# JuliaSmoothOptimizers/LinearOperators.jl

Hardware: AMD Instinct MI355X
Metric: mul! GB/s (frac HBM peak) at n=10^8 fp64; L-BFGS apply/s, 1/2/4/8 GPU (higher is better)
Workload: dtype f64; 1 GPU; opHouseholder(h) 5-arg mul!(res,H,v,1,0), n=100000000 fp64 per GPU (configs[1]); n_per_gpu=100000000, algorithmic_bytes_per_elt=40, devices_visible=1

## Files before the change

linearoperators.jl_amd/csrc/api_ctx.hip:

```cpp
#include "common.h"
#include <vector>

namespace mxlo {
static thread_local char g_err[512] = "";
void set_error(const char *fmt, ...) {
  va_list ap;
  va_start(ap, fmt);
  vsnprintf(g_err, sizeof(g_err), fmt, ap);
  va_end(ap);
}
}

using namespace mxlo;

MXLO_API const char *mxlo_version(void) { return "mxlo 0.1.0 (gfx950)"; }

MXLO_API const char *mxlo_status_string(int32_t s) {
  switch (s) {
    case MXLO_OK: return "ok";
    case MXLO_EINVAL: return "invalid argument";
    case MXLO_ESHAPE: return "shape mismatch";
    case MXLO_EHIP: return "HIP runtime error";
    case MXLO_ENOMEM: return "out of device memory";
    case MXLO_ESTATE: return "wrong variant for this operator state";
// ... 359 lines not shown
MXLO_API int32_t mxlo_ctx_info(mxlo_ctx *ctx, int64_t info[4]) {
  MXLO_REQUIRE(ctx && info, MXLO_EINVAL, "ctx/info is NULL");
  info[0] = ctx->device;
  info[1] = ctx->num_cu;
  info[2] = (int64_t)sizeof(double) * (kMaxRedCols * kMaxRedBlocks + kScalarSlots);
  info[3] = kMaxRedCols;
  return MXLO_OK;
}

MXLO_API int32_t mxlo_ctx_tune(mxlo_ctx *ctx, const char *key, int64_t value) {
  MXLO_REQUIRE(ctx && key, MXLO_EINVAL, "ctx/key is NULL");
  if (!strcmp(key, "blocks_per_cu")) {
    MXLO_REQUIRE(value >= 0 && value <= 64, MXLO_EINVAL, "blocks_per_cu out of range");
    ctx->tune.blocks_per_cu = (int)value;
  } else if (!strcmp(key, "nt_min_bytes")) {
    MXLO_REQUIRE(value >= 0, MXLO_EINVAL, "nt_min_bytes out of range");
    ctx->tune.nt_min_bytes = value;
  } else if (!strcmp(key, "red_blocks_per_cu")) {
    MXLO_REQUIRE(value >= 1 && value * ctx->num_cu <= kMaxRedBlocks, MXLO_EINVAL,
                 "red_blocks_per_cu out of range");
    ctx->tune.red_blocks_per_cu = (int)value;
  } else if (!strcmp(key, "graph_direct_max")) {
    MXLO_REQUIRE(value >= 0 && value <= 4096, MXLO_EINVAL, "graph_direct_max must be in 0..4096 (0: always hipGraphLaunch)");
    ctx->tune.graph_direct_max = (int)value;
  } else if (!strcmp(key, "house_fused")) {
    ctx->tune.house_fused = value != 0;
  } else if (!strcmp(key, "cherm_two_pass")) {
    ctx->tune.cherm_two_pass = value != 0;
  } else if (!strcmp(key, "house_inline_n")) {
    MXLO_REQUIRE(value >= 0, MXLO_EINVAL, "house_inline_n out of range");
    ctx->tune.house_inline_n = value;
  } else if (!strcmp(key, "house_reverse")) {
    ctx->tune.house_reverse = value != 0;
  } else if (!strcmp(key, "lbfgs_inv_mode")) {
    MXLO_REQUIRE(value == MXLO_INV_TWOPASS || value == MXLO_INV_REFORDER, MXLO_EINVAL,
                 "lbfgs_inv_mode must be MXLO_INV_TWOPASS or MXLO_INV_REFORDER");
    ctx->tune.lbfgs_inv_mode = (int)value;
  } else if (!strcmp(key, "gemm_tile")) {
    MXLO_REQUIRE(value == 0 || value == 32 || value == 64 || value == 128 || value == -1, MXLO_EINVAL,
                 "gemm_tile must be 0 (auto), 32, 64, 128 or -1 (generic kernel)");
    ctx->tune.gemm_tile = (int)value;
  } else if (!strcmp(key, "extend_tiles_per_block")) {
    MXLO_REQUIRE(value >= 0 && value <= 1024, MXLO_EINVAL, "extend_tiles_per_block must be in 0..1024 (0 = auto)");
    ctx->tune.extend_tiles_per_block = (int)value;
  } else if (!strcmp(key, "fuse_finalize")) {
    MXLO_REQUIRE(value == 0 || value == 1, MXLO_EINVAL, "fuse_finalize must be 0 or 1");
    ctx->tune.fuse_finalize = (int)value;
  } else if (!strcmp(key, "combine_blocks_per_cu")) {
    MXLO_REQUIRE(value >= 0 && value <= 64, MXLO_EINVAL, "combine_blocks_per_cu out of range");
    ctx->tune.combine_blocks_per_cu = (int)value;
  } else if (!strcmp(key, "qn_fused_max_grid")) {
    MXLO_REQUIRE(value >= 1 && value <= kQnfMaxGrid, MXLO_EINVAL, "qn_fused_max_grid must be in 1..256");
    ctx->tune.qn_fused_max_grid = (int)value;
  } else if (!strcmp(key, "qn_fused_batch12")) {
    MXLO_REQUIRE(value == 0 || value == 1, MXLO_EINVAL, "qn_fused_batch12 must be 0 or 1");
    ctx->tune.qn_fused_batch12 = (int)value;
  } else if (!strcmp(key, "qn_fused_small")) {
    MXLO_REQUIRE(value == 0 || value == 1, MXLO_EINVAL, "qn_fused_small must be 0 or 1");
    ctx->tune.qn_fused_small = (int)value;
  } else if (!strcmp(key, "qn_persist")) {
    MXLO_REQUIRE(value == 0 || value == 1, MXLO_EINVAL, "qn_persist must be 0 or 1");
    ctx->tune.qn_persist = (int)value;
  } else if (!strcmp(key, "qn_persist_min_n")) {
    MXLO_REQUIRE(value >= 1, MXLO_EINVAL, "qn_persist_min_n must be >= 1");
    ctx->tune.qn_persist_min_n = value;
  } else if (!strcmp(key, "qn_persist_max_bytes")) {
// ... 206 lines not shown
```

linearoperators.jl_amd/csrc/common.h:

```cpp
#pragma once
#include <hip/hip_runtime.h>
#include <atomic>

#include <cstdarg>
#include <cstdint>
#include <cstdio>
#include <cstdlib>
#include <cstring>
#include <initializer_list>
#include <type_traits>
#include <utility>
#include <vector>

#include "../../include/mxlo.h"

#define MXLO_API extern "C" __attribute__((visibility("default")))

namespace mxlo {

constexpr int kBlock = 256;
constexpr int kWave = 64;
constexpr int kMaxRedCols = 128;
constexpr int kQnfMaxCols = 40, kQnfMaxGrid = 256;
constexpr int kQnfSlots = kQnfMaxCols * kQnfMaxGrid;
// ... 62 lines not shown
  } while (0)

inline bool mxlo_trace_on() {
  static const bool on = getenv("MXLO_TRACE") != nullptr;
  return on;
}
#define MXLO_LAUNCH_CHECK()                                                                      \
  do {                                                                                           \
    ++mxlo::api_counters().n_launch;                                                             \
    if (mxlo_trace_on()) {                                                                       \
      fprintf(stderr, "[mxlo] launched %s:%d ... ", __FILE__, __LINE__);                         \
      fflush(stderr);                                                                            \
      (void)hipDeviceSynchronize();                                                              \
      fprintf(stderr, "done\n");                                                                 \
    }                                                                                            \
    hipError_t e__ = hipGetLastError();                                                          \
    if (e__ != hipSuccess) {                                                                     \
      mxlo::set_error("kernel launch failed: %s (%s:%d)", hipGetErrorString(e__), __FILE__,      \
                      __LINE__);                                                                 \
      return MXLO_EHIP;                                                                          \
    }                                                                                            \
  } while (0)

struct Tune {
  int blocks_per_cu = 0;
  int extend_tiles_per_block = 0;
  int64_t nt_min_bytes = 256ll << 20;
  int red_blocks_per_cu = 4;
  int graph_direct_max = 16;
  int house_fused_per_cu = 2;
  int house_fused = 1;
  int cherm_two_pass = 0;
  int house_reverse = 1;
  int64_t house_inline_n = 1ll << 23;
  int lbfgs_inv_mode = MXLO_INV_TWOPASS;
  int dots_max_nc = 20;
  int gemm_tile = 0;
  int fuse_finalize = 1;
  int combine_blocks_per_cu = 0;
  int qn_fused_max_grid = 256;
  int qn_fused_batch12 = 1;
  int qn_fused_small = 1;
  int qn_persist = 1;
  int64_t qn_persist_min_n = 1ll << 19;
  int64_t qn_persist_max_bytes = 448ll << 20;
  int qn_persist_reverse = 1;
  int qn_persist_prefetch = 0;
  int qn_persist_lds = 1;
  int qn_persist_lds_pad = 0;
  int64_t qn_persist_min_bytes = 32ll << 20;
  int herm_order = 1;
  int herm_nt = -1;
  int64_t herm_dp_min_bytes = 96ll << 20;
  int64_t herm_nt_min_bytes = 384ll << 20;
  int herm_poll_sleep = 4;
  int herm_strip = 0;
  int herm_lds_pad = 0;
  int herm_single = 1;
  int64_t herm_single_max_n = 0;
  int64_t herm_single_max_bytes = 112ll << 20;
  int kron_fuse = 1;
  int gemv_n_rows = 1;
  int gemvb_n_rows = 1;
  int gemvb_t_lds = 1;
  int combine_reverse = 0;
  int push_wide = 1;
// ... 213 lines not shown
template <typename T>
inline int64_t common_head(std::initializer_list<const void *> ptrs) {
  int64_t mis = -1;
  for (const void *p : ptrs) {
    if (!p) continue;
    int64_t m = (int64_t)((uintptr_t)p & 15u);
    if (m % (int64_t)sizeof(T)) return -1;
    if (mis < 0) mis = m;
    else if (mis != m) return -1;
  }
  if (mis <= 0) return 0;
  return (16 - mis) / (int64_t)sizeof(T);
}

inline int grid_for(const mxlo_ctx *ctx, int64_t work_items, int64_t items_per_block, int per_cu) {
  int64_t need = (work_items + items_per_block - 1) / items_per_block;
  int64_t g = need;
  if (per_cu > 0) {
    const int64_t cap = (int64_t)ctx->num_cu * per_cu;
    if (g > cap) g = cap;
  }
  if (g > 0x7fffffffLL) g = 0x7fffffffLL;
  return (int)(g < 1 ? 1 : g);
}

bool qn_generation(const mxlo_qn *h, int64_t *gen);

int32_t finalize_and_reduce(mxlo_ctx *ctx, int ncols, int nblocks, double *out_dev);
int32_t finalize_and_post(mxlo_ctx *ctx, int ncols, int nblocks, double *out_dev, double *post_dev, unsigned long long seq,
                          const double *extra_src, int extra_n);
int32_t allreduce_hook(mxlo_ctx *ctx, double *dev, int64_t count);
template <typename T>
int32_t panel_dots(mxlo_ctx *ctx, const T *const *cols_host, int ncols, const T *x, int64_t n,
                   double *out_dev);
template <typename T>
int32_t panel_dots_partials(mxlo_ctx *ctx, const T *const *cols_host, int ncols, const T *x, int64_t n, int *nblocks);
template <typename T>
int32_t panel_dots2(mxlo_ctx *ctx, const T *const *cols, int ncols, const T *x1, const T *x2, int64_t n_padded,
                    double *out1, double *out2);
struct PushExtras {
  const double *cp_src = nullptr;
  double *cp_dst = nullptr;
  int cp_n = 0;
  double *post = nullptr;
  unsigned long long post_seq = 0;
};
template <typename T>
int32_t panel_push_pass(mxlo_ctx *ctx, const T *const *cols, int ncols, int slot, int slot_src, const T *x1,
                        const T *x2, int64_t n, int64_t n_padded, T *st1, T *st2, T *stb, double sq, double *out1,
                        double *out2, double *out_x1x2, double *out_x2x2, double *out_bb, double *out_x1x1 = nullptr,
                        const PushExtras *extras = nullptr);

}
```

linearoperators.jl_amd/csrc/leaves.hip:

```cpp
#include "common.h"
#include "stream_kernels.h"

using namespace mxlo;

#define CHECK_COMMON(name)                                                                       \
  MXLO_REQUIRE(ctx != nullptr, MXLO_EINVAL, name ": ctx is NULL");                               \
  MXLO_REQUIRE(dtype == MXLO_F64 || dtype == MXLO_F32, MXLO_EINVAL, name ": bad dtype %d", dtype)

static inline double eff_beta(int32_t dtype, int32_t flags, double beta) {
  return beta_is_f64(dtype == MXLO_F64 ? 8 : 4, flags) ? beta : (double)(float)beta;
}
static inline double eff_alpha(int32_t dtype, int32_t flags, double alpha) {
  return alpha_is_f64(dtype == MXLO_F64 ? 8 : 4, flags) ? alpha : (double)(float)alpha;
}

template <typename T>
static int32_t fill(mxlo_ctx *ctx, T *p, int64_t n, T c) {
  if (n <= 0) return MXLO_OK;
  if (c == T(0)) {
    MXLO_HIP(hipMemsetAsync(p, 0, sizeof(T) * (size_t)n, ctx->stream));
    return MXLO_OK;
  }
  return launch_map<T, 0, false, false>(ctx, p, (const T *)nullptr, (const T *)nullptr, n,
                                        FillOp<T>{c});
// ... 152 lines not shown
template <typename T>
static int32_t ones_mul_t(mxlo_ctx *ctx, T *res, int64_t nrow, const T *v, int64_t ncol,
                          double alpha, double beta, int32_t flags) {
  double *sum = ctx->scalars;
  if (ncol > 0) {
    const int grid = grid_for(ctx, ncol, kBlock * 8, ctx->tune.red_blocks_per_cu);
    hipLaunchKernelGGL((sum_kernel<T>), dim3(grid), dim3(kBlock), 0, ctx->stream, v, ncol,
                       ctx->partials);
    MXLO_LAUNCH_CHECK();
    MXLO_TRY(finalize_and_reduce(ctx, 1, grid, sum));
  } else {
    MXLO_HIP(hipMemsetAsync(sum, 0, sizeof(double), ctx->stream));
  }
  MXLO_TRY(allreduce_hook(ctx, sum, 1));
  return dispatch_ab<T>(beta, flags, [&]<typename CA, typename CB, bool B0>() -> int32_t {
    OnesOp<T, CA, CB, B0> op{(CA)alpha, (CB)beta, sum, (CA)0};
    return launch_map<T, 0, !B0, false>(ctx, res, (const T *)nullptr, (const T *)nullptr, nrow, op);
  });
}

MXLO_API int32_t mxlo_ones_mul(mxlo_ctx *ctx, int32_t dtype, void *res, int64_t nrow,
                               const void *v, int64_t ncol, double alpha, double beta,
                               int32_t flags) {
  CHECK_COMMON("mxlo_ones_mul");
  MXLO_DEVICE_GUARD(ctx);
  MXLO_REQUIRE(nrow >= 0 && ncol >= 0, MXLO_ESHAPE, "mxlo_ones_mul: negative size");
  alpha = eff_alpha(dtype, flags, alpha);
  beta = eff_beta(dtype, flags, beta);
  if (dtype == MXLO_F64)
    return ones_mul_t<double>(ctx, (double *)res, nrow, (const double *)v, ncol, alpha, beta, flags);
  return ones_mul_t<float>(ctx, (float *)res, nrow, (const float *)v, ncol, alpha, beta, flags);
}

template <typename T>
static int32_t householder_apply_t(mxlo_ctx *ctx, T *res, const T *h, const T *v, int64_t n,
                                   double alpha, double beta, int32_t flags, const double *dot) {
  const bool rev = ctx->tune.house_reverse != 0;
  return dispatch_ab<T>(beta, flags, [&]<typename CA, typename CB, bool B0>() -> int32_t {
    HouseholderOp<T, CA, CB, B0> op{(CA)alpha, (CB)beta, dot, T(0)};
    if (rev) return launch_map<T, 2, !B0, true>(ctx, res, h, v, n, op);
    return launch_map<T, 2, !B0, false>(ctx, res, h, v, n, op);
  });
}

namespace {
template <typename T, typename CA, typename CB, bool BETA0, int VPT, bool ALIGNED>
__global__ void __launch_bounds__(kBlock)
householder_fused_kernel(T *__restrict__ res, const T *__restrict__ h, const T *__restrict__ v, int64_t n, CA alpha,
                         CB beta, unsigned long long *__restrict__ slots, unsigned long long ticks,
                         unsigned *__restrict__ fault, int drop) {
  constexpr int VEC = Vec16<T>::N;
  using V = typename Vec16<T>::type;
  const int tid = threadIdx.x, G = (int)gridDim.x, b = (int)blockIdx.x;
  unsigned long long *epoch = slots + 2 * kFusedSlots;
  const unsigned e = (unsigned)__hip_atomic_load(epoch, __ATOMIC_RELAXED, __HIP_MEMORY_SCOPE_AGENT) & 1u;
  unsigned long long *mine = slots + e * kFusedSlots, *other = slots + (1u - e) * kFusedSlots;
  for (int i = b + tid * G; i < kFusedSlots; i += G * kBlock)
    __hip_atomic_store(other + i, kSlotEmpty, __ATOMIC_RELAXED, __HIP_MEMORY_SCOPE_AGENT);

  T hh[VPT][VEC], vv[VPT][VEC];
  double acc = 0.0;
  const int64_t base = (int64_t)b * kBlock * VPT * VEC;
#pragma unroll
  for (int q = 0; q < VPT; ++q) {
    const int64_t i = base + ((int64_t)q * kBlock + tid) * VEC;
    if (ALIGNED && i + VEC <= n) {
      const V a = *reinterpret_cast<const V *>(h + i), c = *reinterpret_cast<const V *>(v + i);
#pragma unroll
      for (int k = 0; k < VEC; ++k) { hh[q][k] = a[k]; vv[q][k] = c[k]; }
    } else {
#pragma unroll
      for (int k = 0; k < VEC; ++k) {
        hh[q][k] = i + k < n ? h[i + k] : T(0);
        vv[q][k] = i + k < n ? v[i + k] : T(0);
      }
// ... 73 lines not shown
      else if (vpt == 4) go.template operator()<4, true>();
      else if (vpt == 8) go.template operator()<8, true>();
      else go.template operator()<16, true>();
    } else {
      if (vpt == 2) go.template operator()<2, false>();
      else if (vpt == 4) go.template operator()<4, false>();
      else if (vpt == 8) go.template operator()<8, false>();
      else go.template operator()<16, false>();
    }
    *launched = fits;
    if (!fits) return MXLO_OK;
    MXLO_LAUNCH_CHECK();
    return MXLO_OK;
  });
}

template <typename T>
static int32_t householder_t(mxlo_ctx *ctx, T *res, const T *h, const T *v, int64_t n,
                             double alpha, double beta, int32_t flags) {
  if (ctx->tune.house_fused && !ctx->allreduce && n > 0 && ctx->fault_dev) {
    MXLO_TRY(fused_fault_check(ctx));
  }
  if (ctx->tune.house_fused && !ctx->allreduce && n > 0 && ctx->fault_dev) {
    const int64_t cap = std::min<int64_t>((int64_t)ctx->num_cu * (ctx->tune.house_fused_per_cu >= 2 ? 2 : 1), kFusedSlots);
    const int64_t cap1 = std::min<int64_t>(ctx->num_cu, kFusedSlots);
    const int vpt = fused_grid<T>(n, 2) <= 16 ? 2 : (fused_grid<T>(n, 4) <= 32 ? 4 : (fused_grid<T>(n, 8) <= cap1 ? 8 : 16));
    if (fused_grid<T>(n, vpt) <= cap) {
      bool launched = false;
      const int32_t st = householder_fused_t<T>(ctx, res, h, v, n, alpha, beta, flags, vpt, &launched);
      if (st != MXLO_OK || launched) return st;
    }
  }
  const T *cols[1] = {h};
  if (!ctx->allreduce && n >= 1 && n <= ctx->tune.house_inline_n) {
    int nb = 0;
    MXLO_TRY(panel_dots_partials<T>(ctx, cols, 1, v, n, &nb));
    const bool rev = ctx->tune.house_reverse != 0;
    return dispatch_ab<T>(beta, flags, [&]<typename CA, typename CB, bool B0>() -> int32_t {
      HouseholderPartialsOp<T, CA, CB, B0> op{(CA)alpha, (CB)beta, ctx->partials, nb, T(0)};
      if (rev) return launch_map<T, 2, !B0, true>(ctx, res, h, v, n, op);
      return launch_map<T, 2, !B0, false>(ctx, res, h, v, n, op);
    });
  }
  double *dot = ctx->scalars;
  MXLO_TRY(panel_dots<T>(ctx, cols, 1, v, n, dot));
  return householder_apply_t<T>(ctx, res, h, v, n, alpha, beta, flags, dot);
}

MXLO_API int32_t mxlo_dot(mxlo_ctx *ctx, int32_t dtype, const void *a, const void *b, int64_t n,
                          double *out_dev) {
  CHECK_COMMON("mxlo_dot");
  MXLO_DEVICE_GUARD(ctx);
  MXLO_REQUIRE(n >= 0 && out_dev && (n == 0 || (a && b)), MXLO_EINVAL, "mxlo_dot: bad argument");
  if (dtype == MXLO_F64) {
    const double *cols[1] = {(const double *)a};
    return panel_dots<double>(ctx, cols, 1, (const double *)b, n, out_dev);
  }
  const float *cols[1] = {(const float *)a};
  return panel_dots<float>(ctx, cols, 1, (const float *)b, n, out_dev);
}

MXLO_API int32_t mxlo_householder_apply(mxlo_ctx *ctx, int32_t dtype, void *res, const void *h,
                                        const void *v, int64_t n, double alpha, double beta,
                                        int32_t flags, const double *dot_dev) {
  CHECK_COMMON("mxlo_householder_apply");
  MXLO_DEVICE_GUARD(ctx);
  MXLO_REQUIRE(n >= 0 && dot_dev && (n == 0 || (res && h && v)), MXLO_EINVAL,
               "mxlo_householder_apply: bad argument");
  MXLO_TRY(stage_alias(ctx, res, n * (dtype == MXLO_F64 ? 8 : 4), &v, n * (dtype == MXLO_F64 ? 8 : 4), true,
                       "mxlo_householder_apply"));
  alpha = eff_alpha(dtype, flags, alpha);
  beta = eff_beta(dtype, flags, beta);
  if (dtype == MXLO_F64)
    return householder_apply_t<double>(ctx, (double *)res, (const double *)h, (const double *)v, n,
                                       alpha, beta, flags, dot_dev);
  return householder_apply_t<float>(ctx, (float *)res, (const float *)h, (const float *)v, n, alpha,
                                    beta, flags, dot_dev);
}

// ... 681 lines not shown
```

linearoperators.jl_amd/csrc/reductions.hip:

```cpp
#include "common.h"

namespace mxlo {

constexpr int kFuseMaxCols = 4;
constexpr int kFuseMaxGrid = 64;

template <typename T, int NC>
struct ColPtrs {
  const T *p[NC];
};

__device__ __forceinline__ double wave_sum(double v) {
#if defined(__HIP_DEVICE_COMPILE__)
  {
    const int lo = __double2loint(v), hi = __double2hiint(v);
    const auto slo = __builtin_amdgcn_permlane32_swap(lo, lo, false, false);
    const auto shi = __builtin_amdgcn_permlane32_swap(hi, hi, false, false);
    v += __hiloint2double((int)shi[1], (int)slo[1]);
  }
  {
    const int lo = __double2loint(v), hi = __double2hiint(v);
    const auto slo = __builtin_amdgcn_permlane16_swap(lo, lo, false, false);
    const auto shi = __builtin_amdgcn_permlane16_swap(hi, hi, false, false);
    v += __hiloint2double((int)shi[1], (int)slo[1]);
// ... 103 lines not shown
#pragma unroll
  for (int c = 0; c < NC; ++c) {
    const double s = wave_sum(acc[c]);
    if (lane == 0) lds[wave][c] = s;
  }
  __syncthreads();
  if (tid < NC) {
    const double s = ((lds[0][tid] + lds[1][tid]) + (lds[2][tid] + lds[3][tid]));
    if constexpr (FUSE) store_agent(partials + (int64_t)tid * kMaxRedBlocks + blockIdx.x, s);
    else partials[(int64_t)tid * kMaxRedBlocks + blockIdx.x] = s;
  }
  if constexpr (FUSE) {
    __shared__ int last;
    __threadfence();
    __syncthreads();
    if (tid == 0) last = atomicAdd(ticket, 1u) == gridDim.x - 1;
    __syncthreads();
    if (!last) return;
    __threadfence();
    const int nblocks = (int)gridDim.x;
#pragma unroll 1
    for (int c = 0; c < NC; ++c) {
      const double *p = partials + (int64_t)c * kMaxRedBlocks;
      double s = 0.0;
      for (int i = tid; i < nblocks; i += kBlock) s += load_agent(p + i);
      s = wave_sum(s);
      __syncthreads();
      if (lane == 0) lds[wave][0] = s;
      __syncthreads();
      if (tid == 0) out[c] = (lds[0][0] + lds[1][0]) + (lds[2][0] + lds[3][0]);
    }
    if (tid == 0) __hip_atomic_store(ticket, 0u, __ATOMIC_RELAXED, __HIP_MEMORY_SCOPE_AGENT);
  }
}

__global__ void __launch_bounds__(kBlock)
finalize_kernel(const double *__restrict__ partials, int nblocks, double *__restrict__ out) {
  const int c = blockIdx.x, tid = threadIdx.x;
  const double *p = partials + (int64_t)c * kMaxRedBlocks;
  double s = 0.0;
  for (int i = tid; i < nblocks; i += kBlock) s += p[i];
  s = wave_sum(s);
  __shared__ double lds[kBlock / kWave];
  if ((tid & 63) == 0) lds[tid >> 6] = s;
  __syncthreads();
  if (tid == 0) out[c] = (lds[0] + lds[1]) + (lds[2] + lds[3]);
}

int32_t finalize_and_reduce(mxlo_ctx *ctx, int ncols, int nblocks, double *out_dev) {
  hipLaunchKernelGGL(finalize_kernel, dim3(ncols), dim3(kBlock), 0, ctx->stream, ctx->partials,
                     nblocks, out_dev);
  MXLO_LAUNCH_CHECK();
  return MXLO_OK;
}

__global__ void __launch_bounds__(kBlock)
finalize_post_kernel(const double *__restrict__ partials, int nblocks, double *__restrict__ out, double *post,
                     unsigned long long seq, const double *__restrict__ extra_src, int extra_n) {
  const int c = blockIdx.x, tid = threadIdx.x;
  auto post_pair = [&](int i, double v) {
    unsigned long long *slot = reinterpret_cast<unsigned long long *>(post) + 2 * i;
    __hip_atomic_store(slot, (unsigned long long)__double_as_longlong(v), __ATOMIC_RELAXED, __HIP_MEMORY_SCOPE_SYSTEM);
    __threadfence_system();
    __hip_atomic_store(slot + 1, seq, __ATOMIC_RELEASE, __HIP_MEMORY_SCOPE_SYSTEM);
  };
  const double *p = partials + (int64_t)c * kMaxRedBlocks;
// ... 31 lines not shown
template <typename T, int VEC, int NC, bool XVEC>
static int32_t launch_dots(mxlo_ctx *ctx, const T *const *cols, const T *x, int64_t head,
                           int64_t nvec, int64_t n, int *nblocks_out, double *fused_out = nullptr) {
  ColPtrs<T, NC> cp;
  for (int c = 0; c < NC; ++c) cp.p[c] = cols[c];
  constexpr int UNROLL = NC <= 2 ? 4 : (NC <= 6 ? 2 : 1);
  const bool nt = (int64_t)sizeof(T) * n * (NC + 1) >= ctx->tune.nt_min_bytes;
  const int per_cu = (nt && NC <= 2 && ctx->tune.red_blocks_per_cu > 1) ? 1 : ctx->tune.red_blocks_per_cu;
  const int grid = grid_for(ctx, nvec, (int64_t)kBlock * UNROLL, per_cu);
  if constexpr (NC <= kFuseMaxCols) {
    if (fused_out && grid <= kFuseMaxGrid) {
      if (nt)
        hipLaunchKernelGGL((panel_dots_kernel<T, VEC, NC, UNROLL, XVEC, true, true>), dim3(grid), dim3(kBlock), 0,
                           ctx->stream, cp, x, head, nvec, n, ctx->partials, ctx->ticket, fused_out);
      else
        hipLaunchKernelGGL((panel_dots_kernel<T, VEC, NC, UNROLL, XVEC, false, true>), dim3(grid), dim3(kBlock), 0,
                           ctx->stream, cp, x, head, nvec, n, ctx->partials, ctx->ticket, fused_out);
      MXLO_LAUNCH_CHECK();
      *nblocks_out = 0;
      return MXLO_OK;
    }
  }
  if (nt)
    hipLaunchKernelGGL((panel_dots_kernel<T, VEC, NC, UNROLL, XVEC, true>), dim3(grid), dim3(kBlock), 0,
                       ctx->stream, cp, x, head, nvec, n, ctx->partials);
  else
    hipLaunchKernelGGL((panel_dots_kernel<T, VEC, NC, UNROLL, XVEC, false>), dim3(grid), dim3(kBlock), 0,
                       ctx->stream, cp, x, head, nvec, n, ctx->partials);
  MXLO_LAUNCH_CHECK();
  *nblocks_out = grid;
  return MXLO_OK;
}

#define DOTS_CASE(NCV)                                                                           \
  case NCV:                                                                                      \
    if (vec && xvec) return launch_dots<T, Vec16<T>::N, NCV, true>(ctx, cols, x, head, nvec, n, nb, fo); \
    if (vec) return launch_dots<T, Vec16<T>::N, NCV, false>(ctx, cols, x, head, nvec, n, nb, fo); \
    break;

template <typename T>
static int32_t dots_chunk(mxlo_ctx *ctx, const T *const *cols, int nc, const T *x, int64_t n,
                          int *nb, double *fo = nullptr) {
  constexpr int VEC = Vec16<T>::N;
  int64_t head = 0;
  bool vec = n >= 4 * VEC;
  if (vec) {
    int64_t mis = -1;
    for (int c = 0; c < nc && vec; ++c) {
      int64_t m = (int64_t)((uintptr_t)cols[c] & 15u);
      if (m % (int64_t)sizeof(T)) vec = false;
      else if (mis < 0) mis = m;
      else if (mis != m) vec = false;
    }
    if (vec) head = mis == 0 ? 0 : (16 - mis) / (int64_t)sizeof(T);
  }
  const int64_t nvec = vec ? (n - head) / VEC : n;
  const bool xvec = vec && ((((uintptr_t)(x + head)) & 15u) == 0);
  switch (nc) {
    DOTS_CASE(1) DOTS_CASE(2) DOTS_CASE(3) DOTS_CASE(4) DOTS_CASE(5) DOTS_CASE(6) DOTS_CASE(7)
    DOTS_CASE(8) DOTS_CASE(9) DOTS_CASE(10) DOTS_CASE(11) DOTS_CASE(12) DOTS_CASE(13)
    DOTS_CASE(14) DOTS_CASE(15) DOTS_CASE(16) DOTS_CASE(17) DOTS_CASE(18) DOTS_CASE(19)
    DOTS_CASE(20)
    default: break;
  }
  switch (nc) {
    case 1: return launch_dots<T, 1, 1, false>(ctx, cols, x, 0, n, n, nb, fo);
    case 2: return launch_dots<T, 1, 2, false>(ctx, cols, x, 0, n, n, nb, fo);
    case 3: return launch_dots<T, 1, 3, false>(ctx, cols, x, 0, n, n, nb, fo);
    case 4: return launch_dots<T, 1, 4, false>(ctx, cols, x, 0, n, n, nb, fo);
    default: break;
  }
  set_error("dots_chunk: unsupported column count %d", nc);
  return MXLO_EINVAL;
}

template <typename T>
int32_t panel_dots(mxlo_ctx *ctx, const T *const *cols, int ncols, const T *x, int64_t n,
                   double *out_dev) {
  MXLO_REQUIRE(ncols >= 0 && ncols <= kMaxRedCols, MXLO_EINVAL, "panel_dots: %d columns", ncols);
  if (ncols == 0) return MXLO_OK;
  if (n <= 0) {
    MXLO_HIP(hipMemsetAsync(out_dev, 0, sizeof(double) * ncols, ctx->stream));
    return allreduce_hook(ctx, out_dev, ncols);
  }
  constexpr int VEC = Vec16<T>::N;
  int done = 0;
  while (done < ncols) {
    int nc = ncols - done;
    if (nc > ctx->tune.dots_max_nc) nc = ctx->tune.dots_max_nc;
    bool vec = n >= 4 * VEC;
    int64_t mis = -1;
    for (int c = 0; c < nc && vec; ++c) {
      int64_t m = (int64_t)((uintptr_t)cols[done + c] & 15u);
      if (m % (int64_t)sizeof(T) || (mis >= 0 && mis != m)) vec = false;
      mis = m;
    }
    if (!vec && nc > 4) nc = 4;
    int nb = 0;
    const bool fuse = ctx->tune.fuse_finalize && done == 0 && nc == ncols && nc <= kFuseMaxCols;
    MXLO_TRY(dots_chunk<T>(ctx, cols + done, nc, x, n, &nb, fuse ? out_dev : nullptr));
    if (nb > 0) MXLO_TRY(finalize_and_reduce(ctx, nc, nb, out_dev + done));
    done += nc;
  }
  return allreduce_hook(ctx, out_dev, ncols);
}

template <typename T>
int32_t panel_dots_partials(mxlo_ctx *ctx, const T *const *cols, int ncols, const T *x, int64_t n, int *nblocks) {
  MXLO_REQUIRE(ncols >= 1 && ncols <= 4 && n >= 1, MXLO_EINVAL, "panel_dots_partials: bad arguments");
  return dots_chunk<T>(ctx, cols, ncols, x, n, nblocks, nullptr);
}
template int32_t panel_dots_partials<double>(mxlo_ctx *, const double *const *, int, const double *, int64_t, int *);
template int32_t panel_dots_partials<float>(mxlo_ctx *, const float *const *, int, const float *, int64_t, int *);

template <typename T, int NC, int UNROLL, bool NT>
__global__ void __launch_bounds__(kBlock)
panel_dots2_kernel(ColPtrs<T, NC> cols, const T *__restrict__ x1, const T *__restrict__ x2, int64_t nvec,
                   double *__restrict__ partials) {
  constexpr int VEC = Vec16<T>::N;
  using V = typename Vec16<T>::type;
  const int tid = threadIdx.x;
  double a1[NC], a2[NC];
#pragma unroll
  for (int c = 0; c < NC; ++c) a1[c] = a2[c] = 0.0;
  auto ld = [&](const T *p, int64_t i) -> V {
    return NT ? __builtin_nontemporal_load(reinterpret_cast<const V *>(p) + i) : reinterpret_cast<const V *>(p)[i];
  };
  constexpr int64_t CHUNK = (int64_t)kBlock * UNROLL;
  const int64_t nchunks = (nvec + CHUNK - 1) / CHUNK;
  for (int64_t ch = blockIdx.x; ch < nchunks; ch += gridDim.x) {
    const int64_t base = ch * CHUNK + tid;
    V xv1[UNROLL], xv2[UNROLL], cv[UNROLL][NC];
    bool ok[UNROLL];
#pragma unroll
    for (int u = 0; u < UNROLL; ++u) {
      const int64_t i = base + (int64_t)u * kBlock;
      ok[u] = i < nvec;
      if (ok[u]) {
        xv1[u] = ld(x1, i);
        xv2[u] = ld(x2, i);
#pragma unroll
        for (int c = 0; c < NC; ++c) cv[u][c] = ld(cols.p[c], i);
      }
    }
#pragma unroll
    for (int u = 0; u < UNROLL; ++u) {
// ... 280 lines not shown
    }
    hipLaunchKernelGGL(finalize_map_kernel, dim3(2 * NC + 4), dim3(kBlock), 0, ctx->stream, ctx->partials, grid, M);
  };
  switch (ncols) {
    case 1: go.template operator()<1>(); break;
    case 2: go.template operator()<2>(); break;
    case 3: go.template operator()<3>(); break;
    case 4: go.template operator()<4>(); break;
    case 5: go.template operator()<5>(); break;
    case 6: go.template operator()<6>(); break;
    case 7: go.template operator()<7>(); break;
    case 8: go.template operator()<8>(); break;
    case 9: go.template operator()<9>(); break;
    case 10: go.template operator()<10>(); break;
    default: go.template operator()<kPushMaxNC>(); break;
  }
  MXLO_LAUNCH_CHECK();
  return MXLO_OK;
}

template int32_t panel_push_pass<double>(mxlo_ctx *, const double *const *, int, int, int, const double *, const double *,
                                         int64_t, int64_t, double *, double *, double *, double, double *, double *,
                                         double *, double *, double *, double *, const PushExtras *);
template int32_t panel_push_pass<float>(mxlo_ctx *, const float *const *, int, int, int, const float *, const float *,
                                        int64_t, int64_t, float *, float *, float *, double, double *, double *, double *,
                                        double *, double *, double *, const PushExtras *);

template int32_t panel_dots2<double>(mxlo_ctx *, const double *const *, int, const double *, const double *, int64_t,
                                     double *, double *);
template int32_t panel_dots2<float>(mxlo_ctx *, const float *const *, int, const float *, const float *, int64_t,
                                    double *, double *);

template int32_t panel_dots<double>(mxlo_ctx *, const double *const *, int, const double *, int64_t,
                                    double *);
template int32_t panel_dots<float>(mxlo_ctx *, const float *const *, int, const float *, int64_t,
                                   double *);

}
```

linearoperators.jl_amd/csrc/stream_kernels.h:

```cpp
#pragma once
#include "common.h"

namespace mxlo {

template <bool NT, typename V>
__device__ __forceinline__ V ldg(const V *p) {
  if constexpr (NT) return __builtin_nontemporal_load(p);
  else return *p;
}
template <bool NT, typename V>
__device__ __forceinline__ void stg(V *p, V v) {
  if constexpr (NT) __builtin_nontemporal_store(v, p);
  else *p = v;
}

template <typename T, int VEC>
struct VecOf {
  using type = T;
};
template <>
struct VecOf<double, 2> {
  using type = f64x2;
};
template <>
// ... 109 lines not shown
  constexpr int VEC = Vec16<T>::N;
  const int64_t head0 = common_head<T>({res, NIN >= 1 ? in0 : nullptr, NIN >= 2 ? in1 : nullptr});
  const int64_t streamed = (int64_t)sizeof(T) * n * (1 + NIN + (READ_RES ? 1 : 0));
  const bool nt = streamed >= ctx->tune.nt_min_bytes;
  auto grid_of = [&](int64_t items) {
    const int64_t need = (items + (int64_t)kBlock * kStreamUnroll - 1) / ((int64_t)kBlock * kStreamUnroll);
    int64_t g = need;
    if (ctx->tune.blocks_per_cu > 0) {
      const int64_t cap = (int64_t)ctx->num_cu * ctx->tune.blocks_per_cu;
      if (g > cap) g = cap;
    }
    if (g > 0x7fffffffLL) g = 0x7fffffffLL;
    return (int)(g < 1 ? 1 : g);
  };
  if (head0 >= 0 && n >= 4 * VEC) {
    const int64_t head = head0 < n ? head0 : n;
    const int64_t nvec = (n - head) / VEC;
    const int grid = grid_of(nvec);
    if (nt)
      hipLaunchKernelGGL((map_kernel<T, VEC, kStreamUnroll, NIN, READ_RES, REVERSE, true, Op>), dim3(grid),
                         dim3(kBlock), 0, ctx->stream, res, in0, in1, head, nvec, n, op);
    else
      hipLaunchKernelGGL((map_kernel<T, VEC, kStreamUnroll, NIN, READ_RES, REVERSE, false, Op>), dim3(grid),
                         dim3(kBlock), 0, ctx->stream, res, in0, in1, head, nvec, n, op);
  } else {
    const int grid = grid_of(n);
    hipLaunchKernelGGL((map_kernel<T, 1, kStreamUnroll, NIN, READ_RES, REVERSE, false, Op>), dim3(grid),
                       dim3(kBlock), 0, ctx->stream, res, in0, in1, (int64_t)0, n, n, op);
  }
  MXLO_LAUNCH_CHECK();
  return MXLO_OK;
}

template <typename CA, typename CB>
using Wider = std::conditional_t<(sizeof(CA) >= sizeof(CB)), CA, CB>;

template <typename T, typename CA, typename CB, bool BETA0>
__device__ __forceinline__ T fin_ab(CA t, CB b, T r) {
  if constexpr (BETA0) return (T)t;
  else {
    using P = Wider<CA, CB>;
    return (T)((P)t + (P)(b * (CB)r));
  }
}

template <typename T, typename CA, typename CB, bool BETA0>
struct DiagOp {
  CA a;
  CB b;
  __device__ void init() {}
  __device__ T operator()(T d, T v, T r) const { return fin_ab<T, CA, CB, BETA0>((a * (CA)d) * (CA)v, b, r); }
};
template <typename T, typename CA, typename CB, bool BETA0>
struct DiagScalarOp {
  CA a;
  CB b;
  const T *dptr;
  CA ad;
  __device__ void init() { ad = a * (CA)(*dptr); }
  __device__ T operator()(T v, T, T r) const { return fin_ab<T, CA, CB, BETA0>(ad * (CA)v, b, r); }
};
template <typename T, typename CA, typename CB, bool BETA0>
struct AxpbyOp {
  CA a;
  CB b;
  __device__ void init() {}
// ... 80 lines not shown
```

Before: 6428 GB/s.

## Keep Householder dot-pass tail cache-resident for the reversed update pass

```diff
diff --git a/linearoperators.jl_amd/csrc/api_ctx.hip b/linearoperators.jl_amd/csrc/api_ctx.hip
--- a/linearoperators.jl_amd/csrc/api_ctx.hip
+++ b/linearoperators.jl_amd/csrc/api_ctx.hip
@@ -415,6 +415,13 @@
     ctx->tune.house_inline_n = value;
   } else if (!strcmp(key, "house_reverse")) {
     ctx->tune.house_reverse = value != 0;
+  } else if (!strcmp(key, "house_tail_bytes")) {
+    MXLO_REQUIRE(value >= 0, MXLO_EINVAL, "house_tail_bytes out of range");
+    ctx->tune.house_tail_bytes = value;
+  } else if (!strcmp(key, "house_tail_store_nt")) {
+    ctx->tune.house_tail_store_nt = value != 0;
+  } else if (!strcmp(key, "house_tail_dots_nt")) {
+    ctx->tune.house_tail_dots_nt = value != 0;
   } else if (!strcmp(key, "lbfgs_inv_mode")) {
     MXLO_REQUIRE(value == MXLO_INV_TWOPASS || value == MXLO_INV_REFORDER, MXLO_EINVAL,
                  "lbfgs_inv_mode must be MXLO_INV_TWOPASS or MXLO_INV_REFORDER");
diff --git a/linearoperators.jl_amd/csrc/common.h b/linearoperators.jl_amd/csrc/common.h
--- a/linearoperators.jl_amd/csrc/common.h
+++ b/linearoperators.jl_amd/csrc/common.h
@@ -118,6 +118,9 @@
   int house_fused = 1;
   int cherm_two_pass = 0;
   int house_reverse = 1;
+  int64_t house_tail_bytes = 128ll << 20;
+  int house_tail_store_nt = 1;
+  int house_tail_dots_nt = 0;
   int64_t house_inline_n = 1ll << 23;
   int lbfgs_inv_mode = MXLO_INV_TWOPASS;
   int dots_max_nc = 20;
@@ -397,9 +400,10 @@
 int32_t allreduce_hook(mxlo_ctx *ctx, double *dev, int64_t count);
 template <typename T>
 int32_t panel_dots(mxlo_ctx *ctx, const T *const *cols_host, int ncols, const T *x, int64_t n,
-                   double *out_dev);
-template <typename T>
-int32_t panel_dots_partials(mxlo_ctx *ctx, const T *const *cols_host, int ncols, const T *x, int64_t n, int *nblocks);
+                   double *out_dev, int64_t nc1_tail_bytes = 0);
+template <typename T>
+int32_t panel_dots_partials(mxlo_ctx *ctx, const T *const *cols_host, int ncols, const T *x, int64_t n, int *nblocks,
+                            int64_t nc1_tail_bytes = 0);
 template <typename T>
 int32_t panel_dots2(mxlo_ctx *ctx, const T *const *cols, int ncols, const T *x1, const T *x2, int64_t n_padded,
                     double *out1, double *out2);
diff --git a/linearoperators.jl_amd/csrc/leaves.hip b/linearoperators.jl_amd/csrc/leaves.hip
--- a/linearoperators.jl_amd/csrc/leaves.hip
+++ b/linearoperators.jl_amd/csrc/leaves.hip
@@ -208,15 +208,32 @@
   return ones_mul_t<float>(ctx, (float *)res, nrow, (const float *)v, ncol, alpha, beta, flags);
 }
 
+template <typename T, bool READ_RES, typename Op>
+static int32_t householder_update(mxlo_ctx *ctx, T *res, const T *h, const T *v, int64_t n, int64_t tail_bytes, Op op) {
+  if (tail_bytes > 0 && launch_map2_split<T, READ_RES>(ctx, res, h, v, n, tail_bytes, ctx->tune.house_tail_store_nt != 0, op)) {
+    MXLO_LAUNCH_CHECK();
+    return MXLO_OK;
+  }
+  if (ctx->tune.house_reverse != 0) return launch_map<T, 2, READ_RES, true>(ctx, res, h, v, n, op);
+  return launch_map<T, 2, READ_RES, false>(ctx, res, h, v, n, op);
+}
+
 template <typename T>
 static int32_t householder_apply_t(mxlo_ctx *ctx, T *res, const T *h, const T *v, int64_t n,
-                                   double alpha, double beta, int32_t flags, const double *dot) {
-  const bool rev = ctx->tune.house_reverse != 0;
+                                   double alpha, double beta, int32_t flags, const double *dot, int64_t tail_bytes = 0) {
   return dispatch_ab<T>(beta, flags, [&]<typename CA, typename CB, bool B0>() -> int32_t {
     HouseholderOp<T, CA, CB, B0> op{(CA)alpha, (CB)beta, dot, T(0)};
-    if (rev) return launch_map<T, 2, !B0, true>(ctx, res, h, v, n, op);
-    return launch_map<T, 2, !B0, false>(ctx, res, h, v, n, op);
-  });
+    return householder_update<T, !B0>(ctx, res, h, v, n, tail_bytes, op);
+  });
+}
+
+template <typename T>
+static int64_t house_tail_of(const mxlo_ctx *ctx, const T *res, const T *h, const T *v, int64_t n) {
+  const Tune &t = ctx->tune;
+  if (t.house_tail_bytes <= 0 || !t.house_reverse || t.blocks_per_cu != 0) return 0;
+  if ((int64_t)sizeof(T) * n * 2 < t.nt_min_bytes || 2 * t.house_tail_bytes >= (int64_t)sizeof(T) * n) return 0;
+  if (n < 4 * Vec16<T>::N || common_head<T>({res, h, v}) < 0) return 0;
+  return t.house_tail_bytes;
 }
 
 namespace {
@@ -356,19 +373,18 @@
     }
   }
   const T *cols[1] = {h};
+  const int64_t tail = house_tail_of<T>(ctx, res, h, v, n);
   if (!ctx->allreduce && n >= 1 && n <= ctx->tune.house_inline_n) {
     int nb = 0;
-    MXLO_TRY(panel_dots_partials<T>(ctx, cols, 1, v, n, &nb));
-    const bool rev = ctx->tune.house_reverse != 0;
+    MXLO_TRY(panel_dots_partials<T>(ctx, cols, 1, v, n, &nb, ctx->tune.house_tail_dots_nt ? 0 : tail));
     return dispatch_ab<T>(beta, flags, [&]<typename CA, typename CB, bool B0>() -> int32_t {
       HouseholderPartialsOp<T, CA, CB, B0> op{(CA)alpha, (CB)beta, ctx->partials, nb, T(0)};
-      if (rev) return launch_map<T, 2, !B0, true>(ctx, res, h, v, n, op);
-      return launch_map<T, 2, !B0, false>(ctx, res, h, v, n, op);
+      return householder_update<T, !B0>(ctx, res, h, v, n, tail, op);
     });
   }
   double *dot = ctx->scalars;
-  MXLO_TRY(panel_dots<T>(ctx, cols, 1, v, n, dot));
-  return householder_apply_t<T>(ctx, res, h, v, n, alpha, beta, flags, dot);
+  MXLO_TRY(panel_dots<T>(ctx, cols, 1, v, n, dot, ctx->tune.house_tail_dots_nt ? 0 : tail));
+  return householder_apply_t<T>(ctx, res, h, v, n, alpha, beta, flags, dot, tail);
 }
 
 MXLO_API int32_t mxlo_dot(mxlo_ctx *ctx, int32_t dtype, const void *a, const void *b, int64_t n,
diff --git a/linearoperators.jl_amd/csrc/reductions.hip b/linearoperators.jl_amd/csrc/reductions.hip
--- a/linearoperators.jl_amd/csrc/reductions.hip
+++ b/linearoperators.jl_amd/csrc/reductions.hip
@@ -159,6 +159,70 @@
     }
     if (tid == 0) __hip_atomic_store(ticket, 0u, __ATOMIC_RELAXED, __HIP_MEMORY_SCOPE_AGENT);
   }
+}
+
+template <bool NT, typename T, int VEC, int UNROLL>
+__device__ __forceinline__ void dots1_whole_chunks(const T *__restrict__ col, const T *__restrict__ x, int64_t &ch,
+                                                   int64_t ch_end, int64_t stride, double &acc) {
+  using V = typename Vec16<T>::type;
+  constexpr int64_t CHUNK = (int64_t)kBlock * UNROLL;
+  auto ld = [](const V *p) -> V {
+    if constexpr (NT) return __builtin_nontemporal_load(p);
+    else return *p;
+  };
+  for (; ch < ch_end; ch += stride) {
+    const int64_t base = ch * CHUNK + threadIdx.x;
+    V xv[UNROLL], cv[UNROLL];
+#pragma unroll
+    for (int u = 0; u < UNROLL; ++u) {
+      const int64_t i = base + (int64_t)u * kBlock;
+      xv[u] = ld(reinterpret_cast<const V *>(x) + i);
+      cv[u] = ld(reinterpret_cast<const V *>(col) + i);
+    }
+#pragma unroll
+    for (int u = 0; u < UNROLL; ++u) {
+#pragma unroll
+      for (int e = 0; e < VEC; ++e) acc = fma((double)cv[u][e], (double)xv[u][e], acc);
+    }
+  }
+}
+
+template <typename T, int VEC, int UNROLL>
+__global__ void __launch_bounds__(kBlock)
+panel_dots1_split_kernel(const T *__restrict__ col, const T *__restrict__ x, int64_t head, int64_t nvec, int64_t n,
+                         int64_t ch_split, double *__restrict__ partials) {
+  const int tid = threadIdx.x;
+  double acc = 0.0;
+  constexpr int64_t CHUNK = (int64_t)kBlock * UNROLL;
+  const int64_t nchunks = (nvec + CHUNK - 1) / CHUNK, stride = gridDim.x;
+  const int64_t nwhole = nvec / CHUNK;
+  int64_t ch = blockIdx.x;
+  dots1_whole_chunks<true, T, VEC, UNROLL>(col + head, x + head, ch, ch_split, stride, acc);
+  dots1_whole_chunks<false, T, VEC, UNROLL>(col + head, x + head, ch, nwhole, stride, acc);
+  if (nwhole < nchunks && (nchunks - 1) % stride == (int64_t)blockIdx.x) {
+#pragma unroll 1
+    for (int u = 0; u < UNROLL; ++u) {
+      const int64_t i = nwhole * CHUNK + tid + (int64_t)u * kBlock;
+      if (i < nvec) {
+#pragma unroll 1
+        for (int e = 0; e < VEC; ++e) acc = fma((double)col[head + i * VEC + e], (double)x[head + i * VEC + e], acc);
+      }
+    }
+  }
+  if (blockIdx.x == gridDim.x - 1) {
+    const int64_t tail0 = head + nvec * VEC;
+    const int64_t cnt = head + (n - tail0);
+    if (tid < cnt) {
+      const int64_t i = tid < head ? tid : tail0 + (tid - head);
+      acc = fma((double)col[i], (double)x[i], acc);
+    }
+  }
+  __shared__ double lds[kBlock / kWave];
+  const int wave = tid >> 6, lane = tid & 63;
+  const double s = wave_sum(acc);
+  if (lane == 0) lds[wave] = s;
+  __syncthreads();
+  if (tid == 0) partials[blockIdx.x] = ((lds[0] + lds[1]) + (lds[2] + lds[3]));
 }
 
 __global__ void __launch_bounds__(kBlock)
@@ -256,6 +320,22 @@
   return MXLO_OK;
 }
 
+template <typename T>
+static bool launch_dots1_split(mxlo_ctx *ctx, const T *col, const T *x, int64_t head, int64_t nvec, int64_t n,
+                               int64_t tail_bytes, int *nblocks_out) {
+  constexpr int VEC = Vec16<T>::N, UNROLL = 4;
+  constexpr int64_t CHUNK = (int64_t)kBlock * UNROLL;
+  if ((int64_t)sizeof(T) * n * 2 < ctx->tune.nt_min_bytes) return false;
+  const int64_t nchunks = (nvec + CHUNK - 1) / CHUNK, tail_chunks = tail_bytes / (CHUNK * 16);
+  if (tail_chunks < 1 || tail_chunks >= nchunks) return false;
+  const int per_cu = ctx->tune.red_blocks_per_cu > 1 ? 1 : ctx->tune.red_blocks_per_cu;
+  const int grid = grid_for(ctx, nvec, CHUNK, per_cu);
+  hipLaunchKernelGGL((panel_dots1_split_kernel<T, VEC, UNROLL>), dim3(grid), dim3(kBlock), 0, ctx->stream, col, x, head,
+                     nvec, n, nchunks - tail_chunks, ctx->partials);
+  *nblocks_out = grid;
+  return true;
+}
+
 #define DOTS_CASE(NCV)                                                                           \
   case NCV:                                                                                      \
     if (vec && xvec) return launch_dots<T, Vec16<T>::N, NCV, true>(ctx, cols, x, head, nvec, n, nb, fo); \
@@ -264,7 +344,7 @@
 
 template <typename T>
 static int32_t dots_chunk(mxlo_ctx *ctx, const T *const *cols, int nc, const T *x, int64_t n,
-                          int *nb, double *fo = nullptr) {
+                          int *nb, double *fo = nullptr, int64_t nc1_tail_bytes = 0) {
   constexpr int VEC = Vec16<T>::N;
   int64_t head = 0;
   bool vec = n >= 4 * VEC;
@@ -280,6 +360,10 @@
   }
   const int64_t nvec = vec ? (n - head) / VEC : n;
   const bool xvec = vec && ((((uintptr_t)(x + head)) & 15u) == 0);
+  if (nc == 1 && nc1_tail_bytes > 0 && xvec && launch_dots1_split<T>(ctx, cols[0], x, head, nvec, n, nc1_tail_bytes, nb)) {
+    MXLO_LAUNCH_CHECK();
+    return MXLO_OK;
+  }
   switch (nc) {
     DOTS_CASE(1) DOTS_CASE(2) DOTS_CASE(3) DOTS_CASE(4) DOTS_CASE(5) DOTS_CASE(6) DOTS_CASE(7)
     DOTS_CASE(8) DOTS_CASE(9) DOTS_CASE(10) DOTS_CASE(11) DOTS_CASE(12) DOTS_CASE(13)
@@ -300,7 +384,7 @@
 
 template <typename T>
 int32_t panel_dots(mxlo_ctx *ctx, const T *const *cols, int ncols, const T *x, int64_t n,
-                   double *out_dev) {
+                   double *out_dev, int64_t nc1_tail_bytes) {
   MXLO_REQUIRE(ncols >= 0 && ncols <= kMaxRedCols, MXLO_EINVAL, "panel_dots: %d columns", ncols);
   if (ncols == 0) return MXLO_OK;
   if (n <= 0) {
@@ -322,7 +406,7 @@
     if (!vec && nc > 4) nc = 4;
     int nb = 0;
     const bool fuse = ctx->tune.fuse_finalize && done == 0 && nc == ncols && nc <= kFuseMaxCols;
-    MXLO_TRY(dots_chunk<T>(ctx, cols + done, nc, x, n, &nb, fuse ? out_dev : nullptr));
+    MXLO_TRY(dots_chunk<T>(ctx, cols + done, nc, x, n, &nb, fuse ? out_dev : nullptr, nc1_tail_bytes));
     if (nb > 0) MXLO_TRY(finalize_and_reduce(ctx, nc, nb, out_dev + done));
     done += nc;
   }
@@ -330,12 +414,13 @@
 }
 
 template <typename T>
-int32_t panel_dots_partials(mxlo_ctx *ctx, const T *const *cols, int ncols, const T *x, int64_t n, int *nblocks) {
+int32_t panel_dots_partials(mxlo_ctx *ctx, const T *const *cols, int ncols, const T *x, int64_t n, int *nblocks,
+                            int64_t nc1_tail_bytes) {
   MXLO_REQUIRE(ncols >= 1 && ncols <= 4 && n >= 1, MXLO_EINVAL, "panel_dots_partials: bad arguments");
-  return dots_chunk<T>(ctx, cols, ncols, x, n, nblocks, nullptr);
-}
-template int32_t panel_dots_partials<double>(mxlo_ctx *, const double *const *, int, const double *, int64_t, int *);
-template int32_t panel_dots_partials<float>(mxlo_ctx *, const float *const *, int, const float *, int64_t, int *);
+  return dots_chunk<T>(ctx, cols, ncols, x, n, nblocks, nullptr, nc1_tail_bytes);
+}
+template int32_t panel_dots_partials<double>(mxlo_ctx *, const double *const *, int, const double *, int64_t, int *, int64_t);
+template int32_t panel_dots_partials<float>(mxlo_ctx *, const float *const *, int, const float *, int64_t, int *, int64_t);
 
 template <typename T, int NC, int UNROLL, bool NT>
 __global__ void __launch_bounds__(kBlock)
@@ -682,8 +767,8 @@
                                     double *, double *);
 
 template int32_t panel_dots<double>(mxlo_ctx *, const double *const *, int, const double *, int64_t,
-                                    double *);
+                                    double *, int64_t);
 template int32_t panel_dots<float>(mxlo_ctx *, const float *const *, int, const float *, int64_t,
-                                   double *);
-
-}
+                                   double *, int64_t);
+
+}
diff --git a/linearoperators.jl_amd/csrc/stream_kernels.h b/linearoperators.jl_amd/csrc/stream_kernels.h
--- a/linearoperators.jl_amd/csrc/stream_kernels.h
+++ b/linearoperators.jl_amd/csrc/stream_kernels.h
@@ -165,6 +165,89 @@
   return MXLO_OK;
 }
 
+template <bool LD_NT, bool ST_NT, typename T, int VEC, int UNROLL, bool READ_RES, typename Op>
+__device__ __forceinline__ void map2_whole_chunk(T *__restrict__ res, const T *__restrict__ in0, const T *__restrict__ in1,
+                                                 int64_t base, const Op &op) {
+  using V = typename VecOf<T, VEC>::type;
+  V *rv = reinterpret_cast<V *>(res);
+  const V *av = reinterpret_cast<const V *>(in0);
+  const V *bv = reinterpret_cast<const V *>(in1);
+  V a[UNROLL], b[UNROLL], r[UNROLL];
+#pragma unroll
+  for (int u = 0; u < UNROLL; ++u) {
+    const int64_t i = base + (int64_t)u * kBlock;
+    a[u] = ldg<LD_NT>(av + i);
+    b[u] = ldg<LD_NT>(bv + i);
+    if constexpr (READ_RES) r[u] = ldg<true>(rv + i);
+  }
+#pragma unroll
+  for (int u = 0; u < UNROLL; ++u) {
+    V o;
+#pragma unroll
+    for (int e = 0; e < VEC; ++e) {
+      const T r0 = READ_RES ? vget<T, VEC>(r[u], e) : T(0);
+      vset<T, VEC>(o, e, op(vget<T, VEC>(a[u], e), vget<T, VEC>(b[u], e), r0));
+    }
+    stg<ST_NT>(rv + base + (int64_t)u * kBlock, o);
+  }
+}
+
+template <typename T, int VEC, int UNROLL, bool READ_RES, bool ST_HEAD_NT, bool ST_TAIL_NT, typename Op>
+__global__ void __launch_bounds__(kBlock)
+map2_split_kernel(T *__restrict__ res, const T *__restrict__ in0, const T *__restrict__ in1, int64_t head, int64_t nvec,
+                  int64_t n, int64_t c_split, Op op) {
+  static_assert(VEC > 1, "vector path only");
+  op.init();
+  const int tid = threadIdx.x;
+  constexpr int64_t CHUNK = (int64_t)kBlock * UNROLL;
+  const int64_t nchunks = (nvec + CHUNK - 1) / CHUNK;
+  const int64_t c = nchunks - 1 - (int64_t)blockIdx.x;
+  const int64_t base = c * CHUNK + tid;
+  if (c < c_split) {
+    asm volatile("; nt region" ::: "memory");
+    map2_whole_chunk<true, ST_HEAD_NT, T, VEC, UNROLL, READ_RES>(res + head, in0 + head, in1 + head, base, op);
+    asm volatile("; nt region end" ::: "memory");
+  } else if ((c + 1) * CHUNK <= nvec) {
+    asm volatile("; default-policy region" ::: "memory");
+    map2_whole_chunk<false, ST_TAIL_NT, T, VEC, UNROLL, READ_RES>(res + head, in0 + head, in1 + head, base, op);
+    asm volatile("; default-policy region end" ::: "memory");
+  } else {
+    const int64_t j0 = head + c * CHUNK * VEC, j1 = head + nvec * VEC;
+#pragma unroll 1
+    for (int64_t j = j0 + tid; j < j1; j += kBlock) res[j] = op(in0[j], in1[j], READ_RES ? res[j] : T(0));
+  }
+  if (blockIdx.x == gridDim.x - 1) {
+    const int64_t tail0 = head + nvec * VEC;
+    const int64_t cnt = head + (n - tail0);
+    if (tid < cnt) {
+      const int64_t i = tid < head ? tid : tail0 + (tid - head);
+      res[i] = op(in0[i], in1[i], READ_RES ? res[i] : T(0));
+    }
+  }
+}
+
+template <typename T, bool READ_RES, typename Op>
+bool launch_map2_split(mxlo_ctx *ctx, T *res, const T *in0, const T *in1, int64_t n, int64_t tail_bytes, bool tail_store_nt,
+                       Op op) {
+  constexpr int VEC = Vec16<T>::N;
+  constexpr int64_t CHUNK = (int64_t)kBlock * kStreamUnroll;
+  const int64_t head0 = common_head<T>({res, in0, in1});
+  if (head0 < 0 || n < 4 * VEC || ctx->tune.blocks_per_cu != 0) return false;
+  if ((int64_t)sizeof(T) * n * (3 + (READ_RES ? 1 : 0)) < ctx->tune.nt_min_bytes) return false;
+  const int64_t head = head0 < n ? head0 : n;
+  const int64_t nvec = (n - head) / VEC;
+  const int64_t nchunks = (nvec + CHUNK - 1) / CHUNK, tail_chunks = tail_bytes / (CHUNK * 16);
+  if (tail_chunks < 1 || tail_chunks >= nchunks || nchunks > 0x7fffffffLL) return false;
+  const int64_t c_split = nchunks - tail_chunks;
+  if (tail_store_nt)
+    hipLaunchKernelGGL((map2_split_kernel<T, VEC, kStreamUnroll, READ_RES, true, true, Op>), dim3((unsigned)nchunks),
+                       dim3(kBlock), 0, ctx->stream, res, in0, in1, head, nvec, n, c_split, op);
+  else
+    hipLaunchKernelGGL((map2_split_kernel<T, VEC, kStreamUnroll, READ_RES, true, false, Op>), dim3((unsigned)nchunks),
+                       dim3(kBlock), 0, ctx->stream, res, in0, in1, head, nvec, n, c_split, op);
+  return true;
+}
+
 template <typename CA, typename CB>
 using Wider = std::conditional_t<(sizeof(CA) >= sizeof(CB)), CA, CB>;
 
```

Measured after the change: 6721 GB/s (median of 3 runs). 4.6% higher.
